# kocurvik/mdrp

Measured on NVIDIA B200. Metric: image_pairs_per_sec, higher is better.
Workload: dtype f64

## Files before the change

mdrp_b200/csrc/repose_b200.cu:

```cuda
#include <cuda.h>
#include <cuda_runtime.h>
#include <algorithm>
#include <cstdio>
#include <cstdlib>
#include <cstring>
#include <string>
#include <vector>

#include "rp_kernels.cuh"

using namespace rp;

namespace {

std::string g_create_error;

struct DevBuf {
    void *p = nullptr;
    size_t cap = 0;
    cudaError_t reserve(size_t bytes) {
        if (bytes <= cap) return cudaSuccess;
        if (p) cudaFree(p);
        p = nullptr;
        cap = 0;
        const size_t want = bytes + bytes / 8 + 256;
        cudaError_t e = cudaMalloc(&p, want);
        if (e == cudaSuccess) cap = want;
        return e;
    }
    void release() {
        if (p) cudaFree(p);
        p = nullptr;
        cap = 0;
    }
    template <class T>
    T *as() const { return (T *)p; }
};

enum { B_OFFS, B_PAIRS, B_PTS64, B_PTS32, B_BEAR, B_SAMPLES, B_MODELS, B_HYPITER, B_SCORE, B_COUNT, B_SEGCNT,
       B_ITEMPFX, B_SCALARS, B_EVENTS, B_NEVENTS, B_LOMODELS, B_LOOFEV, B_LOCOUNT, B_PROBLIST, B_LOSCORE,
       B_LOCNT, B_LOITEMPFX, B_BEST, B_FINSTART, B_FINSCORE, B_FINCNT, B_ONES, B_ONEPFX, B_ENABLE, B_STATS,
       B_PTS32P, B_UB, B_LB, B_FIRSTCNT, B_FIRSTPFX, B_B0, B_S0, B_SURVLIST, B_SURVCNT, B_SURVPFX, B_WAVECUR, B_WAVECNT,
       B_MASK, B_IN_X1, B_IN_X2, B_IN_D1, B_IN_D2, B_IN_CAMS, B_TMP0, B_TMP1, B_TMP2,
       B_MASK_B, B_IN_X1_B, B_IN_X2_B, B_IN_D1_B, B_IN_D2_B, B_IN_CAMS_B, B_TMP0_B, B_TMP1_B,
       B_FEAT, B_TCOUT, B_TCLIST, B_TCLISTCNT, B_TCLISTPFX, B_PAIRCNT, B_TCPFX, B_TCSPLIT,
       B_PAIRFLAGS, B_SUB_IDX, B_SUB_SRC, B_SUB_DST, B_SUB_X1, B_SUB_X2, B_SUB_D1, B_SUB_D2, B_SUB_CAMS, B_SUB_MODELS,
       B_SUB_STATS, B_SUB_MASK, B_NBUF };

struct Scalars {
    int n_items, n_lo_items, n_one_items, n_prob, n_pairs_scalar, any_flag, reserved0, n_first_items;
    int n_surv_items, bound_work, lm_work, score_work;
    unsigned long long point_scores, lm_iters, n_survivors, evaluated_ps;
    long long n_hyp;
    int n_tc_items, n_tcsel_items;
    unsigned long long tc_evaluated, tc_selected, lm_flops;
};

constexpr int N_EVENTS = 26;

}

struct rp_ctx {
    int device = 0;
    int sms = 148;
    std::string err;
    int64_t launches = 0;
    cudaStream_t stream = nullptr;
    cudaStream_t copy_stream = nullptr;
    DevBuf buf[B_NBUF];
    cudaEvent_t ev[N_EVENTS];
    double last_ms[16] = {0};
    double prev_h2d_ms = 0.0, prev_dev_ms = 0.0;
    int64_t last_cnt[16] = {0};
    size_t workspace_budget = (size_t)80 << 30;
    bool prune = true;
    int head = HB;
    bool waves = true;
    int lm_warp = 0xf;
    int head_small = 32;
    int mid_end = 256;
    int mid_ends[4] = {256, 0, 0, 0}, n_mid = 1;
    bool tc = true;
    int tc_two_pass = -115;
    void *encode_tiled = nullptr;
    int ev_cap0 = EV;
    std::vector<int32_t> pair_status;
    int occ_score[4] = {0}, occ_lm[4] = {0};
};

namespace {

#define CK(call)                                                                                     \
    do {                                                                                             \
        cudaError_t e_ = (call);                                                                     \
        if (e_ != cudaSuccess) {                                                                     \
            char b_[512];                                                                            \
            snprintf(b_, sizeof b_, "%s failed at %s:%d: %s", #call, __FILE__, __LINE__,             \
                     cudaGetErrorString(e_));                                                        \
            ctx->err = b_;                                                                           \
            return RP_ERR_CUDA;                                                                      \
        }                                                                                            \
    } while (0)

#define LAUNCHED()                                                                                   \
    do {                                                                                             \
        ctx->launches++;                                                                             \
        CK(cudaGetLastError());                                                                      \
    } while (0)

inline int cdiv(long long a, long long b) { return (int)((a + b - 1) / b); }

int fail(rp_ctx *ctx, int code, const char *msg) {
    if (ctx) ctx->err = msg;
    return code;
}

typedef CUresult (*EncodeTiledFn)(CUtensorMap *, CUtensorMapDataType, cuuint32_t, void *, const cuuint64_t *, const cuuint64_t *,
                                  const cuuint32_t *, const cuuint32_t *, CUtensorMapInterleave, CUtensorMapSwizzle,
                                  CUtensorMapL2promotion, CUtensorMapFloatOOBfill);

int launch_tc(rp_ctx *ctx, const tc::TcArgs &a, float4 *feat, long long n_rows, cudaStream_t st) {
    CUtensorMap tmap;
    const cuuint64_t gdim[2] = {(cuuint64_t)tc::FEAT, (cuuint64_t)std::max<long long>(n_rows, 1)};
    const cuuint64_t gstride[1] = {(cuuint64_t)tc::FEAT * 4};
    const cuuint32_t box[2] = {(cuuint32_t)tc::FEAT, (cuuint32_t)tc::NT};
    const cuuint32_t estr[2] = {1, 1};
    const CUresult cr = ((EncodeTiledFn)ctx->encode_tiled)(&tmap, CU_TENSOR_MAP_DATA_TYPE_FLOAT32, 2, feat, gdim, gstride, box, estr,
                                                           CU_TENSOR_MAP_INTERLEAVE_NONE, CU_TENSOR_MAP_SWIZZLE_128B,
                                                           CU_TENSOR_MAP_L2_PROMOTION_L2_128B, CU_TENSOR_MAP_FLOAT_OOB_FILL_NONE);
    if (cr != CUDA_SUCCESS) {
        ctx->err = "cuTensorMapEncodeTiled failed (" + std::to_string((int)cr) + ")";
        return RP_ERR_CUDA;
    }
    tc::tc_count_kernel<0><<<ctx->sms, tc::THREADS, tc::SMEM_BYTES, st>>>(tmap, a);
    LAUNCHED();
    return RP_OK;
}

template <class K>
int occupancy_grid(rp_ctx *ctx, K kernel, int threads) {
    int nb = 0;
    if (cudaOccupancyMaxActiveBlocksPerMultiprocessor(&nb, kernel, threads, 0) != cudaSuccess || nb < 1) nb = 1;
    return nb * ctx->sms;
}

int launch_score(rp_ctx *ctx, bool pose, bool mask, const ScoreArgs &args, cudaStream_t st) {
    int grid;
    ScoreArgs a = args;
    a.work_counter = &ctx->buf[B_SCALARS].as<Scalars>()->score_work;
    CK(cudaMemsetAsync(a.work_counter, 0, sizeof(int), st));
    if (pose) {
        if (mask) { grid = occupancy_grid(ctx, score_kernel<true, true>, SCORE_THREADS); score_kernel<true, true><<<grid, SCORE_THREADS, 0, st>>>(a); }
        else { grid = occupancy_grid(ctx, score_kernel<true, false>, SCORE_THREADS); score_kernel<true, false><<<grid, SCORE_THREADS, 0, st>>>(a); }
    } else {
        if (mask) { grid = occupancy_grid(ctx, score_kernel<false, true>, SCORE_THREADS); score_kernel<false, true><<<grid, SCORE_THREADS, 0, st>>>(a); }
        else { grid = occupancy_grid(ctx, score_kernel<false, false>, SCORE_THREADS); score_kernel<false, false><<<grid, SCORE_THREADS, 0, st>>>(a); }
    }
    LAUNCHED();
    return RP_OK;
}

int launch_bound(rp_ctx *ctx, bool pose, const BoundArgs &a, cudaStream_t st) {
    CK(cudaMemsetAsync(a.work_counter, 0, sizeof(int), st));
    if (pose) bound_kernel<true><<<occupancy_grid(ctx, bound_kernel<true>, SCORE_THREADS), SCORE_THREADS, 0, st>>>(a);
    else bound_kernel<false><<<occupancy_grid(ctx, bound_kernel<false>, SCORE_THREADS), SCORE_THREADS, 0, st>>>(a);
    LAUNCHED();
    return RP_OK;
}

int launch_lm(rp_ctx *ctx, int variant, const LMArgs &a, long long expected_problems, cudaStream_t st) {
    ctx->launches++;
    (void)expected_problems;
    LMArgs la = a;
    la.work_counter = &ctx->buf[B_SCALARS].as<Scalars>()->lm_work;
    la.warp_kernel = (ctx->lm_warp >> variant) & 1;
    la.warp_single = (ctx->lm_warp >> 4) & 1;
    CK(cudaMemsetAsync(la.work_counter, 0, sizeof(int), st));
    CK((cudaError_t)launch_lm_kernel(ctx->sms, variant, la, st));
    return RP_OK;
}

int launch_solve(rp_ctx *ctx, int variant, const SolveArgs &a, int n_pairs, cudaStream_t st) {
    dim3 grid(a.nseg, n_pairs);
    const bool generic = getenv("RP_SOLVE_GENERIC") != nullptr;
    switch (variant) {
    case RP_CALIB:
        if (generic) solve_kernel<RP_CALIB><<<grid, SOLVE_THREADS, 0, st>>>(a);
        else solve2_kernel<P3PCand><<<grid, SOLVE_THREADS, 0, st>>>(a);
        break;
    case RP_CALIB_SHIFT:
        if (generic) solve_kernel<RP_CALIB_SHIFT><<<grid, SOLVE_THREADS, 0, st>>>(a);
        else solve2_kernel<ShiftCand><<<grid, SOLVE_THREADS, 0, st>>>(a);
        break;
    case RP_SHARED:
        if (generic) solve_kernel<RP_SHARED><<<grid, SOLVE_THREADS, 0, st>>>(a);
        else solve2_kernel<FocalCand><<<grid, SOLVE_THREADS, 0, st>>>(a);
        break;
    default: solve_kernel<RP_VARYING><<<grid, SOLVE_THREADS, 0, st>>>(a); break;
    }
    LAUNCHED();
    return RP_OK;
}

__global__ void valid_ones_kernel(int n_pairs, const PairParams *pairs, int *ones) {
    const int i = blockIdx.x * blockDim.x + threadIdx.x;
    if (i < n_pairs) ones[i] = pairs[i].valid ? 1 : 0;
}

__global__ void stage_points_kernel(int n, const double *x1, const double *x2, double sq_thr, Pt64 *pts64,
                                    float4 *pts32, Bear *bear, PairParams *pair) {
    const int lane = threadIdx.x;
    double Mmax = 0.0, mmax = 0.0;
    for (int k = lane; k < n; k += 32) {
        Pt64 p;
        p.x1_0 = x1[2 * k]; p.x1_1 = x1[2 * k + 1]; p.x2_0 = x2[2 * k]; p.x2_1 = x2[2 * k + 1];
        pts64[k] = p;
        pts32[k] = make_float4((float)p.x1_0, (float)p.x1_1, (float)p.x2_0, (float)p.x2_1);
        const V3 b1 = bearing(p.x1_0, p.x1_1), b2 = bearing(p.x2_0, p.x2_1);
        Bear b;
        b.b1x = b1.x; b.b1y = b1.y; b.b1z = b1.z; b.b2x = b2.x; b.b2y = b2.y; b.b2z = b2.z;
        bear[k] = b;
        const double m1 = fabs(p.x1_0) + fabs(p.x1_1) + 1.0, m2 = fabs(p.x2_0) + fabs(p.x2_1) + 1.0;
        Mmax = fmax(Mmax, m1 * m2);
        mmax = fmax(mmax, fmax(m1, m2));
    }
    Mmax = warp_max(Mmax);
    mmax = warp_max(mmax);
    if (lane == 0) {
        PairParams pp;
        pp.off = 0; pp.n = n; pp.valid = 1;
        pp.sq_thr = sq_thr;
        pp.thr = sqrt(sq_thr) * (1.0 + 1e-15);
        pp.scale_reproj = 0.0; pp.lo_loss_scale = pp.thr; pp.final_loss_scale = pp.thr; pp.nscale = 1.0;
        pp.Mmax = Mmax * 1.000001; pp.mmax = mmax * 1.000001; pp.pbase = 0;
        *pair = pp;
    }
}

struct ChunkIO {
    int n_pairs;
    long long n_points;
    const long long *h_offsets_rel;
    const double *x1, *x2, *d1, *d2, *cams;
    Model *models_out;
    rp_stats *stats_out;
    unsigned char *masks_out;
};

int run_chunk(rp_ctx *ctx, int variant, const rp_options &opt, const ChunkIO &io, int iters, int ev_cap,
              std::vector<int> &flags, cudaStream_t st) {
    const int P = io.n_pairs;
    const long long N = io.n_points;
    const bool pose = variant == RP_CALIB || variant == RP_CALIB_SHIFT;
    const int nseg = std::max(1, cdiv(iters, SEG));
    const size_t slots_pp = (size_t)nseg * 4 * SEG;
    const size_t slots = slots_pp * (size_t)P;

    DevBuf *B = ctx->buf;
    CK(B[B_OFFS].reserve(sizeof(long long) * (P + 1)));
    CK(B[B_PAIRS].reserve(sizeof(PairParams) * P));
    CK(B[B_PTS64].reserve(sizeof(Pt64) * std::max<long long>(N, 1)));
    CK(B[B_PTS32].reserve(sizeof(float4) * std::max<long long>(N, 1)));
    CK(B[B_PTS32P].reserve(32 * (size_t)((N + P + 4) / 2 + 1)));
    CK(B[B_BEAR].reserve(sizeof(Bear) * std::max<long long>(N, 1)));
    CK(B[B_SAMPLES].reserve(sizeof(int) * 3 * (size_t)P * std::max(iters, 1)));
    CK(B[B_MODELS].reserve(sizeof(Model) * slots));
    CK(B[B_HYPITER].reserve(sizeof(int) * slots));
    CK(B[B_SCORE].reserve(sizeof(double) * slots));
    CK(B[B_COUNT].reserve(sizeof(int) * slots));
    CK(B[B_SEGCNT].reserve(sizeof(int) * (size_t)P * nseg));
    CK(B[B_ITEMPFX].reserve(sizeof(int) * ((size_t)P * nseg + 1)));
    CK(B[B_SCALARS].reserve(sizeof(Scalars)));
    CK(B[B_EVENTS].reserve(sizeof(int) * (size_t)P * ev_cap));
    CK(B[B_NEVENTS].reserve(sizeof(int) * P));
    CK(B[B_LOMODELS].reserve(sizeof(Model) * (size_t)P * ev_cap));
    CK(B[B_LOOFEV].reserve(sizeof(int) * (size_t)P * ev_cap));
    CK(B[B_LOCOUNT].reserve(sizeof(int) * P));
    CK(B[B_PROBLIST].reserve(sizeof(int) * (size_t)P * ev_cap));
    CK(B[B_LOSCORE].reserve(sizeof(double) * (size_t)P * ev_cap));
    CK(B[B_PAIRFLAGS].reserve(sizeof(int) * P));
    CK(B[B_LOCNT].reserve(sizeof(int) * (size_t)P * ev_cap));
    CK(B[B_LOITEMPFX].reserve(sizeof(int) * (P + 1)));
    CK(B[B_BEST].reserve(sizeof(Model) * P));
    CK(B[B_FINSTART].reserve(sizeof(Model) * P));
    CK(B[B_FINSCORE].reserve(sizeof(double) * P));
    CK(B[B_FINCNT].reserve(sizeof(int) * P));
    CK(B[B_ONES].reserve(sizeof(int) * P));
    CK(B[B_ONEPFX].reserve(sizeof(int) * (P + 1)));
    CK(B[B_ENABLE].reserve(sizeof(int) * P));
    CK(B[B_STATS].reserve(sizeof(rp_stats) * P));
    if (ctx->prune) {
        CK(B[B_UB].reserve(sizeof(int) * slots));
        CK(B[B_LB].reserve(sizeof(float) * slots));
        CK(B[B_SURVLIST].reserve(sizeof(int) * slots));
        CK(B[B_FIRSTCNT].reserve(sizeof(int) * P));
        CK(B[B_FIRSTPFX].reserve(sizeof(int) * (P + 1)));
        CK(B[B_B0].reserve(sizeof(int) * P));
        CK(B[B_S0].reserve(sizeof(double) * P));
        CK(B[B_SURVCNT].reserve(sizeof(int) * P));
        CK(B[B_WAVECUR].reserve(sizeof(int) * P)); CK(B[B_WAVECNT].reserve(sizeof(int) * P));
        CK(B[B_SURVPFX].reserve(sizeof(int) * (P + 1)));
    }
    const bool use_tc = ctx->prune && ctx->tc;
    if (use_tc) {
        CK(B[B_FEAT].reserve(128 * (size_t)std::max<long long>(N, 1) + 128 * tc::NT));
        CK(B[B_TCOUT].reserve(sizeof(int) * slots));
        CK(B[B_TCLIST].reserve(sizeof(int) * slots));
        CK(B[B_TCLISTCNT].reserve(sizeof(int) * P));
        CK(B[B_TCLISTPFX].reserve(sizeof(int) * (P + 1)));
        CK(B[B_PAIRCNT].reserve(sizeof(int) * P));
        CK(B[B_TCSPLIT].reserve(sizeof(int) * P));
        CK(B[B_TCPFX].reserve(sizeof(int) * (P + 1)));
    }

    Scalars *sc = B[B_SCALARS].as<Scalars>();
    PairParams *pairs = B[B_PAIRS].as<PairParams>();
    Pt64 *pts64 = B[B_PTS64].as<Pt64>();
    float4 *pts32 = B[B_PTS32].as<float4>();
    Bear *bear = B[B_BEAR].as<Bear>();
    int *samples = B[B_SAMPLES].as<int>();
    Model *models = B[B_MODELS].as<Model>();
    int *hyp_iter = B[B_HYPITER].as<int>();
    double *score = B[B_SCORE].as<double>();
    int *count = B[B_COUNT].as<int>();
    int *seg_count = B[B_SEGCNT].as<int>();
    int *item_prefix = B[B_ITEMPFX].as<int>();

    Scalars h_sc;
    memset(&h_sc, 0, sizeof h_sc);
    h_sc.n_pairs_scalar = P;
    CK(cudaMemcpyAsync(sc, &h_sc, sizeof h_sc, cudaMemcpyHostToDevice, st));
    CK(cudaMemcpyAsync(B[B_OFFS].p, io.h_offsets_rel, sizeof(long long) * (P + 1), cudaMemcpyHostToDevice, st));

    cudaEvent_t *ev = ctx->ev;
    CK(cudaEventRecord(ev[0], st));
    {
        PrepareArgs a;
        a.variant = variant; a.n_pairs = P; a.offsets = B[B_OFFS].as<long long>();
        a.x1 = io.x1; a.x2 = io.x2; a.cams = io.cams;
        a.max_epipolar_error = opt.max_epipolar_error; a.max_reproj_error = opt.max_reproj_error;
        a.loss_scale = opt.loss_scale;
        a.pts64 = pts64; a.pts32 = pts32; a.bear = bear; a.pairs = pairs; a.pts32p = B[B_PTS32P].as<float>();
        prepare_kernel<<<cdiv((long long)P * 32, 256), 256, 0, st>>>(a);
        LAUNCHED();
        if (use_tc && N > 0) {
            tc::tc_features_kernel<<<cdiv(N, 256), 256, 0, st>>>(N, pts32, B[B_FEAT].as<float4>());
            LAUNCHED();
        }
    }
    CK(cudaEventRecord(ev[1], st));
    if (iters > 0) {
        if (opt.progressive_sampling)
            sample_prosac_kernel<<<cdiv((long long)P * 32, 256), 256, 0, st>>>(
                P, iters, pairs, opt.seed, (unsigned long long)std::max<int64_t>(opt.max_prosac_iterations, 0), samples);
        else
            sample_kernel<<<cdiv((long long)P * 32, 256), 256, 0, st>>>(P, iters, pairs, opt.seed, samples);
        LAUNCHED();
    }
    CK(cudaEventRecord(ev[2], st));
    {
        SolveArgs a;
        a.variant = variant; a.iters = iters; a.nseg = nseg; a.pairs = pairs; a.samples = samples;
        a.pts64 = pts64; a.d1 = io.d1; a.d2 = io.d2; a.models = models; a.hyp_iter = hyp_iter; a.seg_count = seg_count;
        int rc = launch_solve(ctx, variant, a, P, st);
        if (rc) return rc;
    }
    CK(cudaEventRecord(ev[3], st));
    ScoreArgs sa;
    sa.pairs = pairs; sa.pts32 = pts32; sa.pts64 = pts64; sa.bear = bear; sa.mask = nullptr;
    sa.slot_list = nullptr; sa.list_stride = 0;
    build_items_kernel<<<1, 1024, 0, st>>>(P * nseg, seg_count, item_prefix, &sc->n_items, &sc->n_hyp);
    LAUNCHED();
    if (!ctx->prune) {
        sa.n_groups = P * nseg; sa.grp_stride = 4 * SEG; sa.grp_per_pair = nseg; sa.grp_cnt = seg_count;
        sa.item_prefix = item_prefix; sa.n_items = &sc->n_items; sa.models = models; sa.score = score; sa.count = count;
        sa.point_scores = &sc->point_scores;
        int rc = launch_score(ctx, pose, false, sa, st);
        if (rc) return rc;
    } else {
        const bool mid = use_tc && ctx->mid_end > ctx->head_small && ctx->mid_end > 0;
        const int head = mid ? ctx->head_small : ctx->head;
        int *first_cnt = B[B_FIRSTCNT].as<int>();
        first_count_kernel<<<cdiv(P, 256), 256, 0, st>>>(P, nseg, seg_count, first_cnt, head);
        LAUNCHED();
        build_items_kernel<<<1, 1024, 0, st>>>(P, first_cnt, B[B_FIRSTPFX].as<int>(), &sc->n_first_items, nullptr);
        LAUNCHED();
        sa.n_groups = P; sa.grp_stride = (int)slots_pp; sa.grp_per_pair = 1; sa.grp_cnt = first_cnt;
        sa.item_prefix = B[B_FIRSTPFX].as<int>(); sa.n_items = &sc->n_first_items; sa.models = models;
        sa.score = score; sa.count = count; sa.point_scores = &sc->point_scores;
        int rc = launch_score(ctx, pose, false, sa, st);
        if (rc) return rc;
        pair_bounds_kernel<<<cdiv((long long)P * 32, 256), 256, 0, st>>>(P, nseg, first_cnt, score, count,
                                                                       B[B_B0].as<int>(), B[B_S0].as<double>());
        LAUNCHED();
        auto cascade = [&](int start, int limit, int two_pass, cudaEvent_t ev_tc, cudaEvent_t ev_bound) -> int {
            BoundArgs ba;
            ba.n_groups = P * nseg; ba.grp_stride = 4 * SEG; ba.grp_per_pair = nseg; ba.grp_cnt = seg_count;
            ba.item_prefix = item_prefix; ba.n_items = &sc->n_items; ba.pairs = pairs; ba.models = models; ba.pts32p = B[B_PTS32P].as<ulonglong2>();
            ba.ub = B[B_UB].as<int>(); ba.lb = B[B_LB].as<float>(); ba.point_scores = &sc->point_scores;
            ba.B0 = B[B_B0].as<int>(); ba.S0 = B[B_S0].as<double>();
            ba.evaluated = &sc->evaluated_ps;
            ba.work_counter = &sc->bound_work; ba.head = start;
            ba.slot_list = nullptr; ba.list_stride = 0;
            if (use_tc) {
                range_count_kernel<<<cdiv(P, 256), 256, 0, st>>>(P, nseg, seg_count, start, limit, B[B_PAIRCNT].as<int>());
                LAUNCHED();
                build_items_kernel<<<1, 1024, 0, st>>>(P, B[B_PAIRCNT].as<int>(), B[B_TCPFX].as<int>(), &sc->n_tc_items, nullptr, tc::TILE_MODELS);
                LAUNCHED();
                tc::TcArgs ta;
                memset(&ta, 0, sizeof ta);
                ta.n_pairs = P; ta.nseg = nseg; ta.pairs = pairs; ta.seg_count = seg_count; ta.item_prefix = B[B_TCPFX].as<int>();
                ta.n_items = &sc->n_tc_items; ta.models = models; ta.out = B[B_TCOUT].as<int>(); ta.pose = pose ? 1 : 0;
                ta.evaluated = &sc->tc_evaluated; ta.first = start;
                ta.two_pass = two_pass; ta.pass = 0; ta.split = B[B_TCSPLIT].as<int>();
                if (two_pass) {
                    tc::tc_split_kernel<<<cdiv(P, 256), 256, 0, st>>>(P, pairs, ba.B0, ba.S0, two_pass, B[B_TCSPLIT].as<int>());
                    LAUNCHED();
                }
                int rc = launch_tc(ctx, ta, B[B_FEAT].as<float4>(), N, st);
                if (rc) return rc;
                TcSelectArgs sel;
                sel.n_pairs = P; sel.nseg = nseg; sel.head = start; sel.limit = limit; sel.pairs = pairs; sel.seg_count = seg_count;
                sel.out = B[B_TCOUT].as<int>(); sel.B0 = ba.B0; sel.S0 = ba.S0; sel.ub = ba.ub; sel.lb = ba.lb;
                sel.list = B[B_TCLIST].as<int>(); sel.list_cnt = B[B_TCLISTCNT].as<int>();
                sel.n_selected = two_pass ? nullptr : &sc->tc_selected;
                tc_select_kernel<<<cdiv((long long)P * 32, 256), 256, 0, st>>>(sel);
                LAUNCHED();
                if (two_pass) {
                    build_items_kernel<<<1, 1024, 0, st>>>(P, B[B_TCLISTCNT].as<int>(), B[B_TCPFX].as<int>(), &sc->n_tc_items, nullptr, tc::TILE_MODELS);
                    LAUNCHED();
                    ta.pass = 1; ta.first = 0; ta.list = B[B_TCLIST].as<int>(); ta.list_cnt = B[B_TCLISTCNT].as<int>(); ta.list_stride = (int)slots_pp;
                    rc = launch_tc(ctx, ta, B[B_FEAT].as<float4>(), N, st);
                    if (rc) return rc;
                    sel.n_selected = &sc->tc_selected;
                    tc_select_list_kernel<<<cdiv((long long)P * 32, 256), 256, 0, st>>>(sel);
                    LAUNCHED();
                }
                if (ev_tc) CK(cudaEventRecord(ev_tc, st));
                build_items_kernel<<<1, 1024, 0, st>>>(P, B[B_TCLISTCNT].as<int>(), B[B_TCLISTPFX].as<int>(), &sc->n_tcsel_items, nullptr);
                LAUNCHED();
                ba.n_groups = P; ba.grp_stride = (int)slots_pp; ba.grp_per_pair = 1; ba.grp_cnt = B[B_TCLISTCNT].as<int>();
                ba.item_prefix = B[B_TCLISTPFX].as<int>(); ba.n_items = &sc->n_tcsel_items;
                ba.slot_list = B[B_TCLIST].as<int>(); ba.list_stride = (int)slots_pp;
            }
            int rc = launch_bound(ctx, pose, ba, st);
            if (rc) return rc;
            if (ev_bound) CK(cudaEventRecord(ev_bound, st));
            PruneArgs pa;
            pa.n_pairs = P; pa.nseg = nseg; pa.seg_count = seg_count; pa.ub = ba.ub; pa.lb = ba.lb;
            pa.B0 = B[B_B0].as<int>(); pa.S0 = B[B_S0].as<double>(); pa.score = score; pa.count = count; pa.head = start; pa.limit = limit;
            pa.surv_list = B[B_SURVLIST].as<int>(); pa.surv_cnt = B[B_SURVCNT].as<int>();
            pa.n_survivors = ctx->waves ? nullptr : &sc->n_survivors;
            prune_kernel<<<cdiv((long long)P * 32, 256), 256, 0, st>>>(pa);
            LAUNCHED();
            ScoreArgs sv = sa;
            sv.item_prefix = B[B_SURVPFX].as<int>(); sv.n_items = &sc->n_surv_items;
            sv.slot_list = pa.surv_list; sv.list_stride = (int)slots_pp; sv.point_scores = nullptr;
            WaveArgs wa;
            wa.n_pairs = P; wa.slots_pp = slots_pp; wa.surv_list = pa.surv_list; wa.surv_cnt = pa.surv_cnt;
            wa.cursor = B[B_WAVECUR].as<int>(); wa.wave_cnt = B[B_WAVECNT].as<int>(); wa.ub = ba.ub; wa.lb = ba.lb;
            wa.B = B[B_B0].as<int>(); wa.S = B[B_S0].as<double>(); wa.score = score; wa.count = count;
            wa.n_exact = &sc->n_survivors;
            if (!ctx->waves) {
                build_items_kernel<<<1, 1024, 0, st>>>(P, pa.surv_cnt, B[B_SURVPFX].as<int>(), &sc->n_surv_items, nullptr);
                LAUNCHED();
                sv.grp_cnt = pa.surv_cnt;
                rc = launch_score(ctx, pose, false, sv, st);
                if (rc) return rc;
                if (limit) {
                    CK(cudaMemsetAsync(wa.cursor, 0, sizeof(int) * P, st));
                    CK(cudaMemcpyAsync(wa.wave_cnt, pa.surv_cnt, sizeof(int) * P, cudaMemcpyDeviceToDevice, st));
                    wa.wave_size = 0; wa.first = 0; wa.n_exact = nullptr;
                    wave_select_kernel<<<cdiv((long long)P * 32, 256), 256, 0, st>>>(wa);
                    LAUNCHED();
                }
            } else {
                CK(cudaMemsetAsync(wa.cursor, 0, sizeof(int) * P, st));
                static const int WAVES[] = {8, 16, 32, 64, 0x7fffffff};
                for (int k = 0; k < 5; ++k) {
                    wa.wave_size = WAVES[k]; wa.first = k == 0;
                    wave_select_kernel<<<cdiv((long long)P * 32, 256), 256, 0, st>>>(wa);
                    LAUNCHED();
                    build_items_kernel<<<1, 1024, 0, st>>>(P, wa.wave_cnt, B[B_SURVPFX].as<int>(), &sc->n_surv_items, nullptr);
                    LAUNCHED();
                    sv.grp_cnt = wa.wave_cnt;
                    rc = launch_score(ctx, pose, false, sv, st);
                    if (rc) return rc;
                }
                if (limit) {
                    wa.wave_size = 0; wa.first = 0; wa.n_exact = nullptr;
                    wave_select_kernel<<<cdiv((long long)P * 32, 256), 256, 0, st>>>(wa);
// ... 837 lines not shown
```

mdrp_b200/csrc/rp_kernels.cuh:

```cuda
#pragma once
#include <cuda_runtime.h>
#include "rp_types.cuh"
#include "rp_solvers.cuh"
#include "rp_score.cuh"
#include "rp_lm_kernel.cuh"
#include "rp_tc.cuh"

namespace rp {

struct PrepareArgs {
    int variant;
    int n_pairs;
    const long long *offsets;
    const double *x1, *x2;
    const double *cams;
    double max_epipolar_error, max_reproj_error, loss_scale;
    Pt64 *pts64;
    float4 *pts32;
    float *pts32p;
    Bear *bear;
    PairParams *pairs;
};

RP_D void store_interleaved(float *pts32p, long long pbase, int k, float x1x, float x1y, float x2x, float x2y) {
// ... 103 lines not shown
    return (uint32_t)z;
}
RP_D uint32_t draw_index(uint64_t &state, uint64_t n) {
    state += 0x9e3779b97f4a7c15ULL;
    const int32_t v = (int32_t)splitmix_int(state);
    return (uint32_t)((uint64_t)(int64_t)v % n);
}

__global__ void sample_kernel(int n_pairs, int iters, const PairParams *pairs, uint64_t seed, int *samples) {
    const int warp = (blockIdx.x * blockDim.x + threadIdx.x) >> 5;
    const int lane = threadIdx.x & 31;
    if (warp >= n_pairs) return;
    const PairParams pp = pairs[warp];
    if (!pp.valid) return;
    const uint64_t n = (uint64_t)pp.n;
    const uint64_t G = 0x9e3779b97f4a7c15ULL;
    int *out = samples + (size_t)warp * iters * 3;
    uint64_t base = seed;
    for (int it0 = 0; it0 < iters; it0 += 32) {
        const int group = min(32, iters - it0);
        int done = 0;
        while (done < group) {
            uint64_t st = base + 3ULL * G * (uint64_t)(lane >= done ? lane - done : 0);
            const uint64_t st0 = st;
            const uint32_t i0 = draw_index(st, n), i1 = draw_index(st, n), i2 = draw_index(st, n);
            const bool active = lane >= done && lane < group;
            const bool dup = active && (i1 == i0 || i2 == i0 || i2 == i1);
            const unsigned m = __ballot_sync(0xffffffffu, dup);
            const int first = m ? (__ffs(m) - 1) : group;
            if (active && lane < first) {
                int *o = out + (size_t)(it0 + lane) * 3;
                o[0] = (int)i0; o[1] = (int)i1; o[2] = (int)i2;
            }
            if (first < group) {
                uint64_t s2 = st0;
                if (lane == first) {
                    uint32_t s[3];
                    for (int i = 0; i < 3; ++i) {
                        bool ok = false;
                        while (!ok) {
                            s[i] = draw_index(s2, n);
                            ok = true;
                            for (int j = 0; j < i; ++j) if (s[i] == s[j]) ok = false;
                        }
                    }
                    int *o = out + (size_t)(it0 + lane) * 3;
                    o[0] = (int)s[0]; o[1] = (int)s[1]; o[2] = (int)s[2];
                }
                base = __shfl_sync(0xffffffffu, s2, first);
                done = first + 1;
            } else {
                base = base + 3ULL * G * (uint64_t)(group - done);
                done = group;
            }
        }
    }
}

struct ProsacState {
    unsigned long long subset_sz;
    unsigned long long gidx;
    unsigned long long gval;
    double T_n;
};

RP_D void prosac_init(ProsacState &ps, unsigned long long num_data, unsigned long long max_prosac) {
    double T_n = (double)max_prosac;
    for (unsigned long long i = 0; i < 3; ++i) T_n *= (double)(3 - i) / (double)(num_data - i);
    ps.subset_sz = 3; ps.gidx = 2; ps.gval = 1; ps.T_n = T_n;
}
RP_D void prosac_advance(ProsacState &ps, unsigned long long k, unsigned long long num_data, unsigned long long max_prosac) {
    if (k < max_prosac && k > ps.gval && ps.subset_sz < num_data) {
        const unsigned long long n = ps.subset_sz;
        const double T_next = ((double)n + 1.0) * ps.T_n / (((double)n + 1.0) - 3.0);
        ps.gval = (unsigned long long)((double)ps.gval + ceil(T_next - ps.T_n));
        ps.T_n = T_next;
        ps.gidx = n;
        ps.subset_sz = n + 1;
    }
}

__global__ void sample_prosac_kernel(int n_pairs, int iters, const PairParams *pairs, uint64_t seed,
                                     unsigned long long max_prosac, int *samples) {
    const int warp = (blockIdx.x * blockDim.x + threadIdx.x) >> 5;
    const int lane = threadIdx.x & 31;
    if (warp >= n_pairs) return;
    const PairParams pp = pairs[warp];
    if (!pp.valid) return;
    const uint64_t n = (uint64_t)pp.n;
    const uint64_t G = 0x9e3779b97f4a7c15ULL;
    int *out = samples + (size_t)warp * iters * 3;
    uint64_t base = seed;
    ProsacState ps;
    prosac_init(ps, n, max_prosac);
    for (int it0 = 0; it0 < iters; it0 += 32) {
        const int group = min(32, iters - it0);
        const long long np_ll = (long long)max_prosac - 1 - (long long)it0;
        const int n_prosac = (int)max(0ll, min((long long)group, np_ll));
        unsigned long long my_sz = 3;
        for (int l = 0; l < n_prosac; ++l) {
            if (l == lane) my_sz = ps.subset_sz;
            prosac_advance(ps, (unsigned long long)(it0 + l) + 2ull, n, max_prosac);
        }
        const bool prosac = lane < n_prosac;
        const uint64_t mod = prosac ? my_sz - 1 : n;
        int done = 0;
        while (done < group) {
            const int lp = max(lane, done);
            const int pro_before = max(0, min(lp, n_prosac) - min(done, n_prosac));
            const uint64_t draws_before = 2ULL * (uint64_t)pro_before + 3ULL * (uint64_t)(lp - done - pro_before);
            uint64_t st = base + G * draws_before;
            const uint64_t st0 = st;
            const uint32_t i0 = draw_index(st, mod), i1 = draw_index(st, mod);
            const uint32_t i2 = prosac ? (uint32_t)(my_sz - 1) : draw_index(st, mod);
            const bool active = lane >= done && lane < group;
            const bool dup = active && (i1 == i0 || (!prosac && (i2 == i0 || i2 == i1)));
            const unsigned m = __ballot_sync(0xffffffffu, dup);
            const int first = m ? (__ffs(m) - 1) : group;
            if (active && lane < first) {
                int *o = out + (size_t)(it0 + lane) * 3;
                o[0] = (int)i0; o[1] = (int)i1; o[2] = (int)i2;
            }
            if (first < group) {
                uint64_t s2 = st0;
                if (lane == first) {
                    uint32_t s[3];
                    const int nd = prosac ? 2 : 3;
                    for (int i = 0; i < nd; ++i) {
                        bool ok = false;
                        while (!ok) {
                            s[i] = draw_index(s2, mod);
                            ok = true;
                            for (int j = 0; j < i; ++j) if (s[i] == s[j]) ok = false;
                        }
                    }
                    if (prosac) s[2] = (uint32_t)(my_sz - 1);
                    int *o = out + (size_t)(it0 + lane) * 3;
                    o[0] = (int)s[0]; o[1] = (int)s[1]; o[2] = (int)s[2];
                }
                base = __shfl_sync(0xffffffffu, s2, first);
                done = first + 1;
            } else {
                const int pro_rest = max(0, min(group, n_prosac) - min(done, n_prosac));
                base = base + G * (2ULL * (uint64_t)pro_rest + 3ULL * (uint64_t)(group - done - pro_rest));
                done = group;
            }
        }
    }
}

struct SolveArgs {
    int variant, iters, nseg;
    const PairParams *pairs;
    const int *samples;
    const Pt64 *pts64;
    const double *d1, *d2;
    Model *models;
    int *hyp_iter;
    int *seg_count;
};

template <int VARIANT>
__global__ void __launch_bounds__(SOLVE_THREADS, RP_SOLVE_MIN_BLOCKS) solve_kernel(SolveArgs a) {
    const int seg = blockIdx.x, pair = blockIdx.y;
    const PairParams pp = a.pairs[pair];
    __shared__ int warp_tot[SOLVE_THREADS / 32];
    __shared__ int running_s;
    const int tid = threadIdx.x, lane = tid & 31, wid = tid >> 5;
    const size_t slot0 = ((size_t)pair * a.nseg + seg) * (size_t)(4 * SEG);
    if (tid == 0) running_s = 0;
    __syncthreads();
    if (!pp.valid) {
        if (tid == 0) a.seg_count[pair * a.nseg + seg] = 0;
        return;
    }
    for (int round = 0; round < SEG / SOLVE_THREADS; ++round) {
        const int it = seg * SEG + round * SOLVE_THREADS + tid;
        ModelSet ms;
        ms.n = 0;
        if (it < a.iters) {
            const int *s = a.samples + ((size_t)pair * a.iters + it) * 3;
            Triplet t;
#pragma unroll
            for (int i = 0; i < 3; ++i) {
                const long long g = pp.off + s[i];
                const Pt64 p = a.pts64[g];
                t.p1[i] = v3(p.x1_0, p.x1_1, 1.0);
                t.p2[i] = v3(p.x2_0, p.x2_1, 1.0);
                t.d1[i] = a.d1[g];
                t.d2[i] = a.d2[g];
            }
            if (VARIANT == RP_CALIB) solve_calib_scale(t, ms);
            else if (VARIANT == RP_CALIB_SHIFT) solve_calib_shift(t, ms);
            else if (VARIANT == RP_SHARED) solve_shared_focal(t, ms);
            else solve_varying_focal(t, ms);
        }
        int incl = ms.n;
#pragma unroll
        for (int o = 1; o < 32; o <<= 1) {
            const int v = __shfl_up_sync(0xffffffffu, incl, o);
            if (lane >= o) incl += v;
        }
        if (lane == 31) warp_tot[wid] = incl;
        __syncthreads();
        int wbase = 0, total = 0;
#pragma unroll
        for (int w = 0; w < SOLVE_THREADS / 32; ++w) {
            const int v = warp_tot[w];
            if (w < wid) wbase += v;
            total += v;
        }
        const int running = running_s;
        const size_t dst = slot0 + running + wbase + (incl - ms.n);
        if (ms.n > 0) { a.models[dst] = ms.m[0]; a.hyp_iter[dst] = it; }
        if (ms.n > 1) { a.models[dst + 1] = ms.m[1]; a.hyp_iter[dst + 1] = it; }
        if (ms.n > 2) { a.models[dst + 2] = ms.m[2]; a.hyp_iter[dst + 2] = it; }
        if (ms.n > 3) { a.models[dst + 3] = ms.m[3]; a.hyp_iter[dst + 3] = it; }
        __syncthreads();
        if (tid == 0) running_s = running + total;
        __syncthreads();
    }
    if (tid == 0) a.seg_count[pair * a.nseg + seg] = running_s;
}

constexpr int SOLVE_QCAP = 4 * SOLVE_THREADS + SOLVE_THREADS;

RP_D Triplet load_triplet(const SolveArgs &a, const PairParams &pp, int pair, int it) {
    const int *s = a.samples + ((size_t)pair * a.iters + it) * 3;
    Triplet t;
#pragma unroll
    for (int i = 0; i < 3; ++i) {
        const long long g = pp.off + s[i];
        const Pt64 p = a.pts64[g];
        t.p1[i] = v3(p.x1_0, p.x1_1, 1.0);
        t.p2[i] = v3(p.x2_0, p.x2_1, 1.0);
        t.d1[i] = a.d1[g];
        t.d2[i] = a.d2[g];
    }
    return t;
}

#ifndef RP_SOLVE2_MIN_BLOCKS
#define RP_SOLVE2_MIN_BLOCKS 3
#endif
template <class CAND>
__global__ void __launch_bounds__(SOLVE_THREADS, RP_SOLVE2_MIN_BLOCKS) solve2_kernel(SolveArgs a) {
    const int seg = blockIdx.x, pair = blockIdx.y;
    const PairParams pp = a.pairs[pair];
    __shared__ int warp_tot[SOLVE_THREADS / 32];
    __shared__ CAND qc[SOLVE_QCAP];
    __shared__ int qit[SOLVE_QCAP];
    const int tid = threadIdx.x, lane = tid & 31, wid = tid >> 5;
    const size_t slot0 = ((size_t)pair * a.nseg + seg) * (size_t)(4 * SEG);
    if (!pp.valid) {
        if (tid == 0) a.seg_count[pair * a.nseg + seg] = 0;
        return;
    }
    int head = 0, tail = 0;
    auto drain = [&](int upto) {
        for (int q = head + tid; q < upto; q += SOLVE_THREADS) {
            const int it = qit[q % SOLVE_QCAP];
            const CAND c = qc[q % SOLVE_QCAP];
            const Triplet t = load_triplet(a, pp, pair, it);
            a.models[slot0 + q] = solve_finish(t, c);
            a.hyp_iter[slot0 + q] = it;
        }
        head = upto;
    };
    for (int round = 0; round < SEG / SOLVE_THREADS; ++round) {
        const int it = seg * SEG + round * SOLVE_THREADS + tid;
        CAND c0, c1, c2, c3;
        int n = 0;
        if (it < a.iters) n = solve_roots(load_triplet(a, pp, pair, it), c0, c1, c2, c3);
        int incl = n;
#pragma unroll
        for (int o = 1; o < 32; o <<= 1) {
            const int v = __shfl_up_sync(0xffffffffu, incl, o);
            if (lane >= o) incl += v;
        }
        __syncthreads();
        if (lane == 31) warp_tot[wid] = incl;
        __syncthreads();
        int wbase = 0, total = 0;
#pragma unroll
        for (int w = 0; w < SOLVE_THREADS / 32; ++w) {
            const int v = warp_tot[w];
            if (w < wid) wbase += v;
            total += v;
        }
        const int pos = tail + wbase + (incl - n);
        if (n > 0) { qc[pos % SOLVE_QCAP] = c0; qit[pos % SOLVE_QCAP] = it; }
        if (n > 1) { qc[(pos + 1) % SOLVE_QCAP] = c1; qit[(pos + 1) % SOLVE_QCAP] = it; }
        if (n > 2) { qc[(pos + 2) % SOLVE_QCAP] = c2; qit[(pos + 2) % SOLVE_QCAP] = it; }
        if (n > 3) { qc[(pos + 3) % SOLVE_QCAP] = c3; qit[(pos + 3) % SOLVE_QCAP] = it; }
        tail += total;
        __syncthreads();
        const int full = head + ((tail - head) / SOLVE_THREADS) * SOLVE_THREADS;
        if (full > head) drain(full);
    }
    drain(tail);
    if (tid == 0) a.seg_count[pair * a.nseg + seg] = tail;
}

__global__ void solve_problems_kernel(int variant, long long n, const double *x1h, const double *x2h,
                                      const double *d1, const double *d2, Model *models, int *counts) {
    const long long i = (long long)blockIdx.x * blockDim.x + threadIdx.x;
    if (i >= n) return;
    Triplet t;
#pragma unroll
    for (int k = 0; k < 3; ++k) {
        t.p1[k] = v3(x1h[9 * i + 3 * k], x1h[9 * i + 3 * k + 1], x1h[9 * i + 3 * k + 2]);
        t.p2[k] = v3(x2h[9 * i + 3 * k], x2h[9 * i + 3 * k + 1], x2h[9 * i + 3 * k + 2]);
        t.d1[k] = d1[3 * i + k];
        t.d2[k] = d2[3 * i + k];
    }
    ModelSet ms;
    solve_minimal(variant, t, ms);
    counts[i] = ms.n;
    if (ms.n > 0) models[4 * i] = ms.m[0];
    if (ms.n > 1) models[4 * i + 1] = ms.m[1];
    if (ms.n > 2) models[4 * i + 2] = ms.m[2];
    if (ms.n > 3) models[4 * i + 3] = ms.m[3];
}

__global__ void build_items_kernel(int n_groups, const int *grp_cnt, int *item_prefix, int *n_items,
                                   long long *n_hyp_total, int gran = HB) {
    __shared__ int wtot[32];
    __shared__ long long whyp[32];
    const int lane = threadIdx.x & 31, wid = threadIdx.x >> 5;
    int carry = 0;
    long long hyps = 0;
    for (int base = 0; base < n_groups; base += 1024) {
        const int e = base + threadIdx.x;
        const int c = e < n_groups ? grp_cnt[e] : 0;
        const int v = (c + gran - 1) / gran;
        hyps += c;
        int incl = v;
#pragma unroll
        for (int o = 1; o < 32; o <<= 1) {
            const int t = __shfl_up_sync(0xffffffffu, incl, o);
            if (lane >= o) incl += t;
        }
        __syncthreads();
        if (lane == 31) wtot[wid] = incl;
        __syncthreads();
        if (wid == 0) {
            const int w = wtot[lane];
            int wi = w;
#pragma unroll
            for (int o = 1; o < 32; o <<= 1) {
                const int t = __shfl_up_sync(0xffffffffu, wi, o);
                if (lane >= o) wi += t;
            }
            wtot[lane] = wi - w;
            if (lane == 31) whyp[0] = wi;
        }
        __syncthreads();
        if (e < n_groups) item_prefix[e] = carry + wtot[wid] + incl - v;
        carry += (int)whyp[0];
    }
#pragma unroll
    for (int o = 16; o > 0; o >>= 1) hyps += __shfl_xor_sync(0xffffffffu, hyps, o);
    __syncthreads();
    if (lane == 0) whyp[wid] = hyps;
    __syncthreads();
    if (threadIdx.x == 0) {
        long long tot = 0;
        for (int w = 0; w < 32; ++w) tot += whyp[w];
        item_prefix[n_groups] = carry;
        *n_items = carry;
        if (n_hyp_total) *n_hyp_total = tot;
    }
}

struct ScoreArgs {
    int n_groups, grp_stride, grp_per_pair;
    const int *grp_cnt;
    const int *item_prefix;
    const int *n_items;
    const PairParams *pairs;
    const Model *models;
    const float4 *pts32;
    const Pt64 *pts64;
    const Bear *bear;
    double *score;
    int *count;
    unsigned char *mask;
    unsigned long long *point_scores;
    const int *slot_list;
    int list_stride;
    int *work_counter;
};

struct HypConst {
    M3 E;
    Quat q;
    V3 t;
};

constexpr int QCAP = 32 + 32 * PT;

struct ScoreShared {
    HypConst hc[HB];
    Filter32 hf[HB];
    Cheir32 hch[HB];
    double psum[HB][SCORE_WARPS];
    int pcnt[HB][SCORE_WARPS];
    unsigned queue[SCORE_WARPS][QCAP];
};

template <bool POSE, bool MASK>
__device__ __noinline__ void score_candidates(ScoreShared &sh, const ScoreArgs &a, const PairParams &pp,
                                              unsigned entry, bool active) {
    const int lane = threadIdx.x & 31, wid = threadIdx.x >> 5;
    const unsigned lt_mask = (1u << lane) - 1u;
    const int h = active ? (int)(entry >> 24) : 0;
    const int k = (int)(entry & 0xffffffu);
    bool inl = false;
    double v = 0.0;
    if (active) {
        const long long g = pp.off + k;
        const Pt64 p = a.pts64[g];
        const double r2 = sampson_r2_exact(sh.hc[h].E, p.x1_0, p.x1_1, p.x2_0, p.x2_1);
        inl = r2 < pp.sq_thr;
        if (POSE && inl) {
            const int scr = cheirality32(sh.hch[h], (float)p.x1_0, (float)p.x1_1, (float)p.x2_0, (float)p.x2_1);
            if (scr == 0) {
                const Bear b = a.bear[g];
                inl = cheirality_exact(sh.hc[h].q, sh.hc[h].t, v3(b.b1x, b.b1y, b.b1z), v3(b.b2x, b.b2y, b.b2z));
            } else {
                inl = scr > 0;
            }
        }
        if (inl) {
            v = r2;
            if (MASK) a.mask[g] = 1;
        }
    }
    const unsigned inl_mask = __ballot_sync(0xffffffffu, inl);
    if (inl_mask == 0) return;
    const int h0 = __shfl_sync(0xffffffffu, h, __ffs(inl_mask) - 1);
    if (__all_sync(0xffffffffu, !inl || h == h0)) {
        v = warp_sum(v);
        if (lane == 0) {
            sh.pcnt[h0][wid] += __popc(inl_mask);
            sh.psum[h0][wid] += v;
        }
        __syncwarp();
        return;
    }
    int c = inl ? 1 : 0;
    const int h_prev = __shfl_up_sync(0xffffffffu, h, 1);
    const unsigned heads = __ballot_sync(0xffffffffu, lane == 0 || h != h_prev);
    const int run_start = 31 - __clz(heads & (0xffffffffu >> (31 - lane)));
#pragma unroll
    for (int o = 1; o < 32; o <<= 1) {
        const double vu = __shfl_up_sync(0xffffffffu, v, o);
        const int cu = __shfl_up_sync(0xffffffffu, c, o);
        if (lane - o >= run_start) { v += vu; c += cu; }
    }
    const bool tail = lane == 31 || ((heads >> (lane + 1)) & 1u);
    const bool do_add = tail && c > 0;
    const unsigned add_mask = __ballot_sync(0xffffffffu, do_add);
    unsigned rank = 0;
    if (do_add) rank = __popc(__match_any_sync(add_mask, h) & lt_mask);
    const unsigned max_rank = __reduce_max_sync(0xffffffffu, rank);
    for (unsigned r = 0; r <= max_rank; ++r) {
        if (do_add && rank == r) {
            sh.pcnt[h][wid] += c;
            sh.psum[h][wid] += v;
        }
        __syncwarp();
    }
}

template <bool POSE, bool MASK>
__global__ void __launch_bounds__(SCORE_THREADS) score_kernel(ScoreArgs a) {
    __shared__ ScoreShared sh;
    const int tid = threadIdx.x, lane = tid & 31, wid = tid >> 5;
    const unsigned lt_mask = (1u << lane) - 1u;
    const int n_items = *a.n_items;
    unsigned *q = sh.queue[wid];
    __shared__ int item_s;
    for (;;) {
        __syncthreads();
        if (tid == 0) item_s = atomicAdd(a.work_counter, 1);
        __syncthreads();
        const int item = item_s;
        if (item >= n_items) break;
        int lo = 0, hi = a.n_groups;
        while (hi - lo > 1) {
            const int mid = (lo + hi) >> 1;
            if (a.item_prefix[mid] <= item) lo = mid; else hi = mid;
        }
        const int e = lo;
        const int pair = e / a.grp_per_pair;
        const int h0 = (item - a.item_prefix[e]) * HB;
        const int nh = min(HB, a.grp_cnt[e] - h0);
        const size_t slot0 = (size_t)e * a.grp_stride + h0;
        const PairParams pp = a.pairs[pair];
        __syncthreads();
        size_t my_slot = slot0 + tid;
        if (a.slot_list && tid < nh) my_slot = (size_t)e * a.grp_stride + a.slot_list[(size_t)e * a.list_stride + h0 + tid];
        if (tid < nh) {
            const Model m = a.models[my_slot];
            HypConst c;
            c.E = POSE ? essential_from_motion(m.q, m.t) : fundamental_from_model(m);
            c.q = m.q;
            c.t = m.t;
            sh.hc[tid] = c;
            Filter32 f32 = make_filter32(c.E, pp.thr, pp.Mmax, pp.mmax);
            f32.pad = (isfinite(c.E.r0.x) && isfinite(c.E.r0.y) && isfinite(c.E.r0.z) && isfinite(c.E.r1.x) &&
                       isfinite(c.E.r1.y) && isfinite(c.E.r1.z) && isfinite(c.E.r2.x) && isfinite(c.E.r2.y) &&
                       isfinite(c.E.r2.z)) ? 0.f : 1.f;
            sh.hf[tid] = f32;
            if (POSE) sh.hch[tid] = make_cheir32(m.q, m.t);
        }
        for (int i = tid; i < HB * SCORE_WARPS; i += SCORE_THREADS) {
            (&sh.psum[0][0])[i] = 0.0;
            (&sh.pcnt[0][0])[i] = 0;
        }
        __syncthreads();
        const int n = pp.n;
        const int slice_pts = 32 * PT;
        const int n_slices = (n + slice_pts - 1) / slice_pts;
        int qn = 0;
        for (int sl = wid; sl < n_slices; sl += SCORE_WARPS) {
            float4 p[PT];
            bool valid[PT];
            const int kbase = sl * slice_pts + lane;
#pragma unroll
            for (int j = 0; j < PT; ++j) {
                const int k = kbase + j * 32;
                valid[j] = k < n;
                p[j] = valid[j] ? a.pts32[pp.off + k] : make_float4(0.f, 0.f, 0.f, 0.f);
            }
            for (int h = 0; h < nh; ++h) {
                const Filter32 f = sh.hf[h];
                if (f.pad != 0.f) continue;
                unsigned cand = 0;
#pragma unroll
                for (int j = 0; j < PT; ++j)
                    if (valid[j] && !certain_outlier32(f, p[j].x, p[j].y, p[j].z, p[j].w)) cand |= 1u << j;
                if (__any_sync(0xffffffffu, cand != 0)) {
#pragma unroll
                    for (int j = 0; j < PT; ++j) {
                        const bool c = (cand >> j) & 1u;
                        const unsigned m = __ballot_sync(0xffffffffu, c);
                        if (c) q[qn + __popc(m & lt_mask)] = ((unsigned)h << 24) | (unsigned)(kbase + j * 32);
                        qn += __popc(m);
                    }
                    __syncwarp();
                    while (qn >= 32) {
                        qn -= 32;
                        const unsigned entry = q[qn + lane];
                        __syncwarp();
                        score_candidates<POSE, MASK>(sh, a, pp, entry, true);
                    }
                }
            }
        }
        if (qn > 0) {
            const unsigned entry = lane < qn ? q[lane] : 0u;
            __syncwarp();
            score_candidates<POSE, MASK>(sh, a, pp, entry, lane < qn);
        }
        __syncthreads();
        if (tid < nh) {
            int c = 0;
            double s = 0.0;
#pragma unroll
            for (int w = 0; w < SCORE_WARPS; ++w) { c += sh.pcnt[tid][w]; s += sh.psum[tid][w]; }
            a.count[my_slot] = c;
            a.score[my_slot] = s + pp.sq_thr * (double)(n - c);
        }
        if (a.point_scores && tid == 0) atomicAdd(a.point_scores, (unsigned long long)nh * (unsigned long long)n);
    }
}

struct BoundArgs {
    int n_groups, grp_stride, grp_per_pair;
    const int *grp_cnt;
    const int *item_prefix;
    const int *n_items;
    const PairParams *pairs;
    const Model *models;
    const ulonglong2 *pts32p;
    int *ub;
    float *lb;
    const int *B0;
    const double *S0;
    unsigned long long *point_scores;
    unsigned long long *evaluated;
    int *work_counter;
    int head;
    const int *slot_list;
    int list_stride;
};

#ifndef RP_SOLVE_MIN_BLOCKS
#define RP_SOLVE_MIN_BLOCKS 1
#endif
#ifndef RP_BOUND_MIN_BLOCKS
#define RP_BOUND_MIN_BLOCKS 2
#endif
#ifndef RP_BOUND_BSG
// ... 832 lines not shown
```

Baseline: 80200.

## Stage P3P sample points into shared memory with cp.async double-buffering

Adds a staged solve kernel for the calibrated variant that prefetches the next round's three-point samples (coordinates and depths) into a shared-memory ring using cp.async while the current round solves. The finish step then reads triplets from shared memory rather than re-gathering from global memory. The intent is to hide scattered global gather latency and avoid reloading the same points twice. In exchange it uses more dynamic shared memory, sets function attributes on every launch, and adds an extra barrier, which may lower occupancy.

After: 80220, median of 6. Within noise of the previous version (+0.0%).

```diff
diff --git a/mdrp_b200/csrc/repose_b200.cu b/mdrp_b200/csrc/repose_b200.cu
--- a/mdrp_b200/csrc/repose_b200.cu
+++ b/mdrp_b200/csrc/repose_b200.cu
@@ -185,8 +185,15 @@
     const bool generic = getenv("RP_SOLVE_GENERIC") != nullptr;
     switch (variant) {
     case RP_CALIB:
-        if (generic) solve_kernel<RP_CALIB><<<grid, SOLVE_THREADS, 0, st>>>(a);
-        else solve2_kernel<P3PCand><<<grid, SOLVE_THREADS, 0, st>>>(a);
+        if (generic) {
+            solve_kernel<RP_CALIB><<<grid, SOLVE_THREADS, 0, st>>>(a);
+        } else {
+            CK(cudaFuncSetAttribute(solve2_staged_kernel<P3PCand>, cudaFuncAttributeMaxDynamicSharedMemorySize,
+                                    (int)SOLVE2_DYN_SMEM));
+            CK(cudaFuncSetAttribute(solve2_staged_kernel<P3PCand>, cudaFuncAttributePreferredSharedMemoryCarveout,
+                                    (int)cudaSharedmemCarveoutMaxShared));
+            solve2_staged_kernel<P3PCand><<<grid, SOLVE_THREADS, SOLVE2_DYN_SMEM, st>>>(a);
+        }
         break;
     case RP_CALIB_SHIFT:
         if (generic) solve_kernel<RP_CALIB_SHIFT><<<grid, SOLVE_THREADS, 0, st>>>(a);
diff --git a/mdrp_b200/csrc/rp_kernels.cuh b/mdrp_b200/csrc/rp_kernels.cuh
--- a/mdrp_b200/csrc/rp_kernels.cuh
+++ b/mdrp_b200/csrc/rp_kernels.cuh
@@ -429,6 +429,121 @@
     if (tid == 0) a.seg_count[pair * a.nseg + seg] = tail;
 }
 
+constexpr int SOLVE_RING = 2 * SOLVE_THREADS;
+static_assert(SEG % SOLVE_RING == 0, "the ring slot of iteration it is it % SOLVE_RING");
+
+struct alignas(16) StagedPt {
+    double x1_0, x1_1, x2_0, x2_1, d1, d2;
+};
+struct StagedSample {
+    StagedPt p[3];
+};
+constexpr size_t SOLVE2_DYN_SMEM = sizeof(StagedSample) * SOLVE_RING;
+
+RP_D Triplet staged_triplet(const StagedSample &s) {
+    Triplet t;
+#pragma unroll
+    for (int i = 0; i < 3; ++i) {
+        const StagedPt p = s.p[i];
+        t.p1[i] = v3(p.x1_0, p.x1_1, 1.0);
+        t.p2[i] = v3(p.x2_0, p.x2_1, 1.0);
+        t.d1[i] = p.d1;
+        t.d2[i] = p.d2;
+    }
+    return t;
+}
+
+RP_D void stage_sample(const SolveArgs &a, const PairParams &pp, const int (&idx)[3], StagedSample &dst) {
+#pragma unroll
+    for (int i = 0; i < 3; ++i) {
+        const long long g = pp.off + idx[i];
+        cp_async16(&dst.p[i].x1_0, &a.pts64[g].x1_0);
+        cp_async16(&dst.p[i].x2_0, &a.pts64[g].x2_0);
+        cp_async8(&dst.p[i].d1, a.d1 + g);
+        cp_async8(&dst.p[i].d2, a.d2 + g);
+    }
+    cp_async_commit();
+}
+
+template <class CAND>
+__global__ void __launch_bounds__(SOLVE_THREADS, 2) solve2_staged_kernel(SolveArgs a) {
+    const int seg = blockIdx.x, pair = blockIdx.y;
+    const PairParams pp = a.pairs[pair];
+    __shared__ int warp_tot[SOLVE_THREADS / 32];
+    __shared__ CAND qc[SOLVE_QCAP];
+    __shared__ int qit[SOLVE_QCAP];
+    extern __shared__ StagedSample staged[];
+    const int tid = threadIdx.x, lane = tid & 31, wid = tid >> 5;
+    const size_t slot0 = ((size_t)pair * a.nseg + seg) * (size_t)(4 * SEG);
+    if (!pp.valid) {
+        if (tid == 0) a.seg_count[pair * a.nseg + seg] = 0;
+        return;
+    }
+    constexpr int ROUNDS = SEG / SOLVE_THREADS;
+    const int *smp = a.samples + (size_t)pair * a.iters * 3;
+    int idx[3];
+    auto load_idx = [&](int it) {
+        if (it < a.iters) {
+#pragma unroll
+            for (int i = 0; i < 3; ++i) idx[i] = smp[(size_t)it * 3 + i];
+        }
+    };
+    const int it0 = seg * SEG + tid;
+    load_idx(it0);
+    if (it0 < a.iters) stage_sample(a, pp, idx, staged[it0 % SOLVE_RING]);
+    int head = 0, tail = 0;
+    for (int round = 0; round < ROUNDS; ++round) {
+        const int it = it0 + round * SOLVE_THREADS;
+        const int itn = it + SOLVE_THREADS;
+        if (round + 1 < ROUNDS) load_idx(itn);
+        CAND c0, c1, c2, c3;
+        int n = 0;
+        if (it < a.iters) {
+            cp_async_wait<0>();
+            n = solve_roots(staged_triplet(staged[it % SOLVE_RING]), c0, c1, c2, c3);
+        }
+        int incl = n;
+#pragma unroll
+        for (int o = 1; o < 32; o <<= 1) {
+            const int v = __shfl_up_sync(0xffffffffu, incl, o);
+            if (lane >= o) incl += v;
+        }
+        if (lane == 31) warp_tot[wid] = incl;
+        __syncthreads();
+        int wbase = 0, total = 0;
+#pragma unroll
+        for (int w = 0; w < SOLVE_THREADS / 32; ++w) {
+            const int v = warp_tot[w];
+            if (w < wid) wbase += v;
+            total += v;
+        }
+        const int round_start = tail;
+        const int pos = tail + wbase + (incl - n);
+        if (n > 0) { qc[pos % SOLVE_QCAP] = c0; qit[pos % SOLVE_QCAP] = it; }
+        if (n > 1) { qc[(pos + 1) % SOLVE_QCAP] = c1; qit[(pos + 1) % SOLVE_QCAP] = it; }
+        if (n > 2) { qc[(pos + 2) % SOLVE_QCAP] = c2; qit[(pos + 2) % SOLVE_QCAP] = it; }
+        if (n > 3) { qc[(pos + 3) % SOLVE_QCAP] = c3; qit[(pos + 3) % SOLVE_QCAP] = it; }
+        tail += total;
+        __syncthreads();
+        int upto = head + ((tail - head) / SOLVE_THREADS) * SOLVE_THREADS;
+        if (round + 1 == ROUNDS) upto = tail;
+        else if (upto < round_start) upto = round_start;
+        const bool reads_prev = head < round_start;
+        for (int q = head + tid; q < upto; q += SOLVE_THREADS) {
+            const int qi = qit[q % SOLVE_QCAP];
+            const CAND c = qc[q % SOLVE_QCAP];
+            a.models[slot0 + q] = solve_finish(staged_triplet(staged[qi % SOLVE_RING]), c);
+            a.hyp_iter[slot0 + q] = qi;
+        }
+        head = upto;
+        if (round + 1 < ROUNDS) {
+            if (reads_prev) __syncthreads();
+            if (itn < a.iters) stage_sample(a, pp, idx, staged[itn % SOLVE_RING]);
+        }
+    }
+    if (tid == 0) a.seg_count[pair * a.nseg + seg] = tail;
+}
+
 __global__ void solve_problems_kernel(int variant, long long n, const double *x1h, const double *x2h,
                                       const double *d1, const double *d2, Model *models, int *counts) {
     const long long i = (long long)blockIdx.x * blockDim.x + threadIdx.x;
```
